# aurelienpierreeng/ansel

Hardware: AMD Instinct MI355X
Metric: MPix/s full export pixelpipe (100 MP raw); % MI355X HBM roofline (higher is better)
Workload: dtype f32

## Files before the change

### ansel_amd/csrc/diffuse.hip

```cpp
#include "hip_common.h"

#include <type_traits>
#include "devmath.h"
#include "ieee_inrange.h"
#include "px_colorspaces.h"

#include <math.h>
#include <cstdlib>

namespace ansel
{
int bspline_launch_decompose(int devid, hipStream_t s, const float4 *in, float4 *hf, float4 *lf, int w, int h, int mult,
                             const unsigned *gate = nullptr);
int bspline_launch_decompose3(int devid, hipStream_t s, const void *in, bool in4, float *lf, int w, int h, int mult, unsigned *alpha_flag);
#ifdef ANSEL_HIP_MEASURING
int bspline_launch_decompose2(int devid, hipStream_t s, const float4 *in, float4 *low1, float4 *low2, int w, int h, int mult);
#endif
}
using namespace ansel;

namespace
{

#define DIFFUSE_MAX_SCALES 10
#define BSPLINE_SIGMA 1.0553651328015339f
#define PDE_KAPPA 0.25f

__device__ __forceinline__ float max_first(const float a, const float b) { return a > b ? a : b; }
__device__ __forceinline__ float max_zero(const float v) { return isfinite(v) ? max_first(v, 0.0f) : 0.0f; }
__device__ __forceinline__ int clampi(const int v, const int lo, const int hi) { return v < lo ? lo : (v > hi ? hi : v); }

__device__ __forceinline__ int walk_row(const int b, const int height, const int mult)
{
  if(height <= mult) return b < height ? b : -1;
  const int per_pass = (height + mult - 1) / mult;
  const int row = (b % per_pass) * mult + b / per_pass;
  return row < height ? row : -1;
}

struct pde_args
{
  int width, height, mult;
  float anisotropy[4];
  int kind[4];
  int same02, same13;
  float variance_threshold, regularization;
  float abcd[4], strength;
  int wskip;
  int post_lab;
  float post_m[3][4];
  int approx_div;
  int off;
  const unsigned *gate;
  int gate_sense;
};

#ifdef ANSEL_HIP_MEASURING
#define PDE_APPROX(a) ((a).approx_div != 0)
#define PDE_OFF(a, bit) (((a).off & (bit)) != 0)
#else
#define PDE_APPROX(a) false
#define PDE_OFF(a, bit) false
#endif
__device__ __forceinline__ float div_1ulp(const float x, const float y)
{
  const float r = __builtin_amdgcn_rcpf(y);
  const float q = x * r;
  return __builtin_fmaf(__builtin_fmaf(-y, q, x), r, q);
}

__device__ __forceinline__ float fast_expf(const float x)
{
  const float t = 1065353216.0f + x * 11401300.0f;
  int k = (t > -2147483648.0f && t < 2147483648.0f) ? (int)t : 0;
  k = k > 0 ? k : 0;
  return __int_as_float(k);
}

__device__ __forceinline__ float direction(float gx, float gy, float &cos2, float &sin2, float &cs, const bool approx = false)
{
  const float s2 = gx * gx + gy * gy;
  float mag, inv;
  if(approx)
  {
    mag = __builtin_amdgcn_sqrtf(s2);
    inv = div_1ulp(1.0f, mag + (1.0f - ((mag != 0.0f) ? 1.0f : 0.0f)));
  }
  else if(__builtin_amdgcn_ballot_w64(!ansel_ieee::zero_or_above_2m96(s2)) == 0ull)
  {
    mag = ansel_ieee::sqrt_core(s2);
    inv = ansel_ieee::rcp_core(mag + (1.0f - ((mag != 0.0f) ? 1.0f : 0.0f)));
  }
  else
  {
    mag = sqrtf(s2);
    inv = 1.0f / (mag + (1.0f - ((mag != 0.0f) ? 1.0f : 0.0f)));
  }
  const float nonzero = (mag != 0.0f) ? 1.0f : 0.0f;
  gx = gx * inv + (1.0f - nonzero);
  gy = gy * inv;
  cos2 = gx * gx;
  sin2 = gy * gy;
  cs = gx * gy;
  return mag;
}

struct kernel5
{
  float k0, k1, k2, k3, k4;
};
__device__ __forceinline__ kernel5 order_kernel(const int kind, const float c2, const float cs, const float cos2, const float sin2)
{
  kernel5 w;
  if(kind == 0)
  {
    w.k0 = 0.25f; w.k1 = 0.5f; w.k2 = 0.25f; w.k3 = 0.5f; w.k4 = -3.0f;
  }
  else
  {
    float a00, a11, a01;
    if(kind == 1)
    {
      a00 = cos2 + c2 * sin2;
      a11 = c2 * cos2 + sin2;
      a01 = (c2 - 1.0f) * cs;
    }
    else
    {
      a00 = c2 * cos2 + sin2;
      a11 = cos2 + c2 * sin2;
      a01 = (1.0f - c2) * cs;
    }
    w.k0 = a01 * 0.5f;
    w.k1 = a11;
    w.k2 = -w.k0;
    w.k3 = a00;
    w.k4 = -2.0f * (a00 + a11);
  }
  return w;
}

__device__ __forceinline__ float convolve(const kernel5 w, const float p[9])
{
  float d = 0.0f;
  d = w.k0 * p[0] + d;
  d = w.k1 * p[1] + d;
  d = w.k2 * p[2] + d;
  d = w.k3 * p[3] + d;
  d = w.k4 * p[4] + d;
  d = w.k3 * p[5] + d;
  d = w.k2 * p[6] + d;
  d = w.k1 * p[7] + d;
  d = w.k0 * p[8] + d;
  return d;
}

__device__ __forceinline__ float ratio2(const float h, const float l)
{
  const float safe = max_zero(l - 1e-8f) + 1e-8f;
  const float ratio = h / safe;
  return ratio * ratio;
}
__device__ __forceinline__ float4 ratio2_rgb(const float4 h, const float4 l, const float w_ratio, const bool approx = false)
{
  if(approx)
  {
    const float ax = div_1ulp(h.x, max_zero(l.x - 1e-8f) + 1e-8f), ay = div_1ulp(h.y, max_zero(l.y - 1e-8f) + 1e-8f),
                az = div_1ulp(h.z, max_zero(l.z - 1e-8f) + 1e-8f);
    return make_float4(ax * ax, ay * ay, az * az, w_ratio);
  }
// ... 652 lines not shown
struct diffuse_planes_t
{
  dev_buf_t hf[DIFFUSE_MAX_SCALES], lf[2], tmp[2];
  dev_buf_t mask;
  dev_buf_t inpainted;
  dev_buf_t alpha_flag;
};

struct diffuse_job_t
{
  int devid;
  hipStream_t st;
  const dt_hip_diffuse_data_t *d;
  const dt_hip_lab_data_t *post_lab;
  int w, h, scales, iterations;
  float zoom;
  bool lf_chain;
  bool per_row, no_dma;
  diffuse_planes_t p;
};

static int diffuse_alloc_planes(diffuse_job_t &j, const bool in_place, const bool three)
{
  diffuse_planes_t &p = j.p;
  const size_t plane = (size_t)j.w * j.h * sizeof(float4);
  bool ok = true;
  for(int s = 0; s < j.scales; s++) ok &= (bool)(p.hf[s] = dev_buf_t::alloc(j.devid, plane));
  for(int k = 0; k < ((j.lf_chain && !in_place) ? 1 : 2); k++) ok &= (bool)(p.lf[k] = dev_buf_t::alloc(j.devid, plane));
  for(int k = 0; k < 2 && k < j.iterations - 1; k++) ok &= (bool)(p.tmp[k] = dev_buf_t::alloc(j.devid, plane));
  if(ok && three) ok &= (bool)(p.alpha_flag = dev_buf_t::alloc(j.devid, sizeof(unsigned)));
  if(ok && j.d->threshold > 0.0f)
  {
    p.mask = dev_buf_t::alloc(j.devid, (size_t)j.w * j.h);
    if(!p.tmp[1]) p.tmp[1] = dev_buf_t::alloc(j.devid, plane);
    p.inpainted = dev_buf_t::borrow(p.tmp[1].base());
    ok = p.mask && p.inpainted;
  }
  return ok ? DT_HIP_SUCCESS : DT_HIP_SYSMEM_ALLOCATION;
}

static void pde_args_of_call(pde_args &a, const int w, const int h, const dt_hip_diffuse_data_t *d)
{
  memset(&a, 0, sizeof(a));
  a.width = w;
  a.height = h;
  a.wskip = measuring_env("ANSEL_HIP_PDE_NO_WSKIP") ? 0 : 1;
  const char *const approx_env = measuring_env("ANSEL_HIP_PDE_APPROX_DIV");
  a.approx_div = approx_env && atoi(approx_env) != 0;
  const char *const off_env = measuring_env("ANSEL_HIP_PDE_OFF");
  a.off = off_env ? atoi(off_env) : 0;
  const float user_aniso[4] = { d->anisotropy_first, d->anisotropy_second, d->anisotropy_third, d->anisotropy_fourth };
  for(int k = 0; k < 4; k++)
  {
    a.anisotropy[k] = sqf(user_aniso[k]);
    a.kind[k] = user_aniso[k] == 0.0f ? 0 : (user_aniso[k] > 0.0f ? 1 : 2);
  }
  a.same02 = a.kind[0] == a.kind[2] && a.anisotropy[0] == a.anisotropy[2];
  a.same13 = a.kind[1] == a.kind[3] && a.anisotropy[1] == a.anisotropy[3];
  a.variance_threshold = powf(10.0f, d->variance_threshold);
}

static void pde_args_of_scale(pde_args &a, const diffuse_job_t &j, const int s, const bool last_pass)
{
  const dt_hip_diffuse_data_t *const d = j.d;
  const float regularization = powf(10.0f, d->regularization) - 1.0f;
  const float speed[4] = { d->first, d->second, d->third, d->fourth };
  const float real_radius = sigma_at_step(BSPLINE_SIGMA, (unsigned)s) * j.zoom;
  a.regularization = regularization / 9.0f * sqf(real_radius);
  const float norm = expf(-sqf(real_radius - (float)d->radius_center) / sqf((float)d->radius));
  for(int k = 0; k < 4; k++) a.abcd[k] = speed[k] * PDE_KAPPA * norm;
  a.strength = d->sharpness * norm + 1.0f;
  a.mult = 1 << s;
  a.post_lab = 0;
  if(j.post_lab && last_pass)
  {
    a.post_lab = 1;
    memcpy(a.post_m, j.post_lab->matrix, sizeof(a.post_m));
  }
}

typedef void (*pde_strip_fn)(const float4 *, const float4 *, const float4 *, float4 *, pde_args, int, const unsigned char *, int, int);
typedef void (*pde_strip3_fn)(const float4 *, const float4 *, const float4 *, float4 *, pde_args, int, int, int);

template <int MD> static pde_strip_fn pde_strip_forms(const bool chain, const bool dma)
{
  if(dma) return diffuse_pde_strip<true, MD, true>;
  if(chain) return diffuse_pde_strip<true, MD>;
  return diffuse_pde_strip<false, MD>;
}
static pde_strip_fn pde_strip_kernel(const int mode, const bool chain, const bool dma)
{
  switch(mode)
  {
#define PDE_CASE(MD) \
  case MD: return pde_strip_forms<MD>(chain, dma);
    PDE_MODES(PDE_CASE)
#undef PDE_CASE
    default: return pde_strip_forms<-1>(chain, dma);
  }
}
static pde_strip3_fn pde_strip3_kernel(const int mode, const bool h0_4)
{
  if(mode == PDE_MODE_DEBLUR) return h0_4 ? diffuse_pde_strip3<PDE_MODE_DEBLUR, true> : diffuse_pde_strip3<PDE_MODE_DEBLUR, false>;
  return h0_4 ? diffuse_pde_strip3<PDE_MODE_ISOTROPIC, true> : diffuse_pde_strip3<PDE_MODE_ISOTROPIC, false>;
}

static void pde_strip_launch(const diffuse_job_t &j, const pde_args &a, const bool p3, const bool h0_4, const bool chain,
                             const bool dma, const float4 *h0, const float4 *h1, const float4 *cur, float4 *to,
                             const int final_pass)
{
  const int w = j.w, h = j.h;
  const int classes = h < a.mult ? h : a.mult, per_class = (h + a.mult - 1) / a.mult;
  const int gx = (w + 255) / 256;
  int longest = 32;
#ifdef ANSEL_HIP_MEASURING
  static const char *const strip_env = measuring_env("ANSEL_HIP_PDE_STRIP");
  if(strip_env) longest = atoi(strip_env);
#endif
  const int strip = strip_rows(gx, classes, per_class, longest);
  const int spc = (per_class + strip - 1) / strip;
  size_t ring = (size_t)PDE_RING * (256 + 2 * a.mult) * sizeof(float4);
#ifdef ANSEL_HIP_MEASURING
  static const char *const pad_env = measuring_env("ANSEL_HIP_PDE_LDS_PAD");
  if(pad_env) ring += (size_t)atoi(pad_env);
#endif
  static const bool generic = measuring_env("ANSEL_HIP_PDE_GENERIC") != nullptr;
  const int mode = generic ? -1 : pde_mode_of(a);
  const dim3 sgrid(gx, classes * spc);
  if(p3)
  {
    const size_t lds3 = (size_t)PDE_RING * (256 + 2 * a.mult) * 12 + (size_t)4 * 3 * (64 + 2 * a.mult) * 16;
    pde_strip3_kernel(mode, h0_4)<<<sgrid, 256, lds3, j.st>>>(h0, h1, cur, to, a, final_pass, strip, spc);
    return;
  }
  const size_t lds = dma ? ring + (size_t)4 * 3 * (64 + 2 * a.mult) * sizeof(float4) : ring;
  pde_strip_kernel(mode, chain, dma)<<<sgrid, 256, lds, j.st>>>(h0, h1, cur, to, a, final_pass, j.p.mask.as<unsigned char>(), strip, spc);
}

static int diffuse_iteration(const diffuse_job_t &j, pde_args &a, const bool p3, const bool first, const bool last,
                             const float4 *src, float4 *dst)
{
  const int w = j.w, h = j.h, scales = j.scales;
  float4 *hf[DIFFUSE_MAX_SCALES];
  for(int s = 0; s < DIFFUSE_MAX_SCALES; s++) hf[s] = j.p.hf[s].as<float4>();
  float4 *const lf[2] = { j.p.lf[0].as<float4>(), j.p.lf[1].as<float4>() };
  unsigned *const alpha_flag = j.p.alpha_flag.as<unsigned>();
  const unsigned char *const mask = j.p.mask.as<unsigned char>();
  int err = DT_HIP_SUCCESS;
  const float4 *level = src;
  float4 *residual = lf[0];
  const bool chain = j.lf_chain && (const float4 *)dst != src;
  for(int s = 0; s < scales && err == DT_HIP_SUCCESS; s++)
  {
#ifdef ANSEL_HIP_MEASURING
    static const bool pairs = measuring_env("ANSEL_HIP_BSPLINE_PAIRS") != nullptr;
    if(chain && pairs && s + 1 < scales && (s == 0 || s == 2))
    {
      err = bspline_launch_decompose2(j.devid, j.st, level, hf[s], hf[s + 1], w, h, 1 << s);
      s++;
      level = residual = hf[s];
      continue;
    }
#endif
    float4 *low = chain ? hf[s] : lf[s % 2];
    if(p3) err = bspline_launch_decompose3(j.devid, j.st, level, first && s == 0, (float *)low, w, h, 1 << s, alpha_flag);
    else err = bspline_launch_decompose(j.devid, j.st, level, chain ? nullptr : hf[s], low, w, h, 1 << s, alpha_flag);
    level = low;
    residual = low;
  }
  float4 *pp[2] = { residual == lf[1] ? lf[0] : lf[1], residual };
  const float4 *cur = residual;
  int count = 0;
  for(int s = scales - 1; s >= 0 && err == DT_HIP_SUCCESS; s--, count++)
  {
    pde_args_of_scale(a, j, s, s == 0 && last);
    float4 *to = (s == 0) ? dst : (chain ? (count % 2 == 0 ? lf[0] : hf[s + 1]) : pp[count % 2]);
    {
      launch_scope ls(j.devid, "diffuse_pde");
      if(a.mult <= PDE_SHARED_MULT && !j.per_row)
      {
        const float4 *const h0 = chain ? (s == 0 ? src : hf[s - 1]) : hf[s], *const h1 = chain ? hf[s] : nullptr;
        const bool dma = chain && a.mult <= PDE_DMA_MAX_MULT && !j.no_dma;
        pde_strip_launch(j, a, p3, first && s == 0, chain, dma, h0, h1, cur, to, p3 ? (s == 0 && last) : s == 0);
      }
      else
      {
        const int rows = (h <= a.mult) ? h : ((h + a.mult - 1) / a.mult) * a.mult;
        const dim3 grid(xcd_pad((w + 255) / 256), rows);
        if(a.mult <= PDE_SHARED_MULT)
          diffuse_pde<true><<<grid, 256, (size_t)3 * (256 + 2 * a.mult) * sizeof(float4), j.st>>>(hf[s], cur, to, a, s == 0, mask);
        else
          diffuse_pde<false><<<grid, 256, 0, j.st>>>(hf[s], cur, to, a, s == 0, mask);
      }
    }
    err = check_launch("diffuse_pde");
    cur = to;
  }
  return err;
}

static int diffuse_run(int devid, const dt_hip_piece_t *piece, const dt_hip_diffuse_data_t *d, int first_row, dt_hip_mem_t dev_in,
                       dt_hip_mem_t dev_out, const dt_hip_lab_data_t *post_lab)
{
  if(!valid_device(devid) || !piece || !d || !dev_in || !dev_out) return DT_HIP_INVALID_ARG;
  if(piece->channels != 4)
  {
    set_last_error("diffuse: needs a 4-channel float input");
    return DT_HIP_INVALID_ARG;
  }
  const int w = piece->roi_out.width, h = piece->roi_out.height;
  if(w <= 0 || h <= 0) return DT_HIP_SUCCESS;
  if(!(d->iscale > 0.0f) || !(piece->roi_in.scale > 0.0)) return DT_HIP_INVALID_ARG;
  static const bool per_row_pde = measuring_env("ANSEL_HIP_PDE_PER_ROW") != nullptr;
  static const bool hf_planes = measuring_env("ANSEL_HIP_DIFFUSE_HF_PLANES") != nullptr;
  static const bool no_dma = measuring_env("ANSEL_HIP_PDE_NO_DMA") != nullptr;
  const int it_req = (int)ceilf((float)d->iterations);
  diffuse_job_t j;
  j.devid = devid;
  j.st = stream_of(devid);
  j.d = d;
  j.post_lab = post_lab;
  j.w = w, j.h = h;
  j.scales = scales_of(piece, d);
  j.iterations = it_req > 1 ? it_req : 1;
  j.zoom = (float)(d->iscale / piece->roi_in.scale);
  j.lf_chain = !per_row_pde && !hf_planes && (1 << (j.scales - 1)) <= PDE_SHARED_MULT;
  j.per_row = per_row_pde, j.no_dma = no_dma;
  const int iterations = j.iterations;
  pde_args a;
  pde_args_of_call(a, w, h, d);

  const int mode0 = pde_mode_of(a);
  const bool in_place = iterations == 1 && dev_in == dev_out && !(d->threshold > 0.0f);
  const bool three = j.lf_chain && !no_dma && !(d->threshold > 0.0f) && (1 << (j.scales - 1)) <= PDE_DMA_MAX_MULT &&
                     !(iterations == 1 && dev_in == dev_out) && !measuring_env("ANSEL_HIP_PDE_GENERIC") &&
                     (mode0 == PDE_MODE_DEBLUR || mode0 == PDE_MODE_ISOTROPIC);
  int err = diffuse_alloc_planes(j, in_place, three);
  unsigned *const alpha_flag = j.p.alpha_flag.as<unsigned>();
  if(err == DT_HIP_SUCCESS && alpha_flag && hipMemsetAsync(alpha_flag, 0, sizeof(unsigned), j.st) != hipSuccess) err = DT_HIP_DEFAULT_ERROR;
  const float4 *src = (const float4 *)dev_in;
  if(err == DT_HIP_SUCCESS && j.p.mask)
  {
    const size_t np = (size_t)w * h;
    launch_scope ls(devid, "diffuse_inpaint");
    diffuse_inpaint<<<pixel_grid(np), 256, 0, j.st>>>(src, j.p.inpainted.as<float4>(), j.p.mask.as<unsigned char>(), d->threshold, np,
                                                      (size_t)w, (size_t)first_row * w);
    err = check_launch("diffuse_inpaint");
    src = j.p.inpainted.as<float4>();
  }
  for(int seq = alpha_flag ? 0 : 1; seq < 2 && err == DT_HIP_SUCCESS; seq++)
  {
    const bool p3 = seq == 0;
    a.gate = alpha_flag;
    a.gate_sense = p3 ? 1 : 2;
    if(alpha_flag) src = (const float4 *)dev_in;
    for(int it = 0; err == DT_HIP_SUCCESS && it < iterations; it++)
    {
      float4 *dst = (it == iterations - 1) ? (float4 *)dev_out : j.p.tmp[it % 2].as<float4>();
      err = diffuse_iteration(j, a, p3, it == 0, it == iterations - 1, src, dst);
      src = dst;
    }
  }
  if(alpha_flag)
  {
    if(g_diffuse_probe && err == DT_HIP_SUCCESS
       && hipMemcpyAsync(g_diffuse_probe, alpha_flag, sizeof(unsigned), hipMemcpyDeviceToDevice, j.st) != hipSuccess)
      err = DT_HIP_DEFAULT_ERROR;
  }
  else if(g_diffuse_probe && err == DT_HIP_SUCCESS && hipMemsetAsync(g_diffuse_probe, 0xff, sizeof(unsigned), j.st) != hipSuccess)
    err = DT_HIP_DEFAULT_ERROR;
  return err;
}

}

extern "C" {

int dt_hip_test_diffuse_probe(void *sink)
{
  ansel::g_diffuse_probe = sink;
  return DT_HIP_SUCCESS;
}

void dt_hip_iop_diffuse_tiling(const dt_hip_piece_t *piece, const dt_hip_diffuse_data_t *d, dt_hip_tiling_t *tiling)
{
  const int scales = scales_of(piece, d);
  tiling->factor = 6.0625f + scales;
  tiling->factor_cl = 6.0625f + scales;
  tiling->maxbuf = 1.0f;
  tiling->maxbuf_cl = 1.0f;
  tiling->overhead = 0;
  tiling->overlap = 1 << scales;
  tiling->xalign = 1;
  tiling->yalign = 1;
}

}
```

### ansel_amd/csrc/diffuse_bspline.hip

```cpp
#include "hip_common.h"

#include <cstdlib>

using namespace ansel;

namespace
{

__device__ __forceinline__ float max_first(const float a, const float b) { return a > b ? a : b; }
__device__ __forceinline__ int clampi(const int v, const int lo, const int hi) { return v < lo ? lo : (v > hi ? hi : v); }

__device__ __forceinline__ float tap5(const float a, const float b, const float c, const float d, const float e)
{
  const float s = 0.0625f * a + 0.25f * b + 0.375f * c + 0.25f * d + 0.0625f * e;
  return max_first(0.0f, s);
}
__device__ __forceinline__ float4 tap5(const float4 a, const float4 b, const float4 c, const float4 d, const float4 e)
{
  return make_float4(tap5(a.x, b.x, c.x, d.x, e.x), tap5(a.y, b.y, c.y, d.y, e.y), tap5(a.z, b.z, c.z, d.z, e.z),
                     tap5(a.w, b.w, c.w, d.w, e.w));
}

__device__ __forceinline__ int walk_row(const int b, const int height, const int mult)
{
// ... 130 lines not shown
    if(more && own) n1 = in[BS_ROW(kk + 3) + col];
    if(more && second) n2 = in[BS_ROW(kk + 3) + col2];
    float4 *const V = vert[kk & 1];
    if(own) V[(k + 2) * R + r] = tap5(a, b, c, d, e);
    if(second) V[slot2] = tap5(a2, b2, c2, d2, e2);
    __syncthreads();
    if(own)
    {
      float4 t[5];
#pragma unroll
      for(int s = -2; s <= 2; s++)
      {
        const int cc = col + s * mult;
        t[s + 2] = cc < 0 ? V[(T + 4) * R] : (cc > width - 1 ? V[(T + 4) * R + 1] : V[(k + s + 2) * R + r]);
      }
      const float4 low = tap5(t[0], t[1], t[2], t[3], t[4]);
      const size_t o = (size_t)row * width + col;
      lf[o] = low;
      if(hf) nt_store(hf + o, make_float4(c.x - low.x, c.y - low.y, c.z - low.z, c.w - low.w));
    }
    a = b;
    b = c;
    c = d;
    d = e;
    e = n1;
    a2 = b2;
    b2 = c2;
    c2 = d2;
    d2 = e2;
    e2 = n2;
  }
#undef BS_ROW
}

struct bs_px3
{
  float x, y, z;
};
__device__ __forceinline__ bs_px3 tap5(const bs_px3 a, const bs_px3 b, const bs_px3 c, const bs_px3 d, const bs_px3 e)
{
  return { tap5(a.x, b.x, c.x, d.x, e.x), tap5(a.y, b.y, c.y, d.y, e.y), tap5(a.z, b.z, c.z, d.z, e.z) };
}
template <int R, int T, bool IN4>
__global__ __launch_bounds__(256) void bspline_decompose_strip3(const void *__restrict__ in_v, bs_px3 *__restrict__ lf,
                                                                const int width, const int height, const int strip,
                                                                const int strips_per_class, unsigned *__restrict__ alpha_flag)
{
  static_assert(R * T == 256, "a workgroup's columns: one span of 256");
  constexpr int mult = R;
  if(!IN4 && *alpha_flag != 0u) return;
  __shared__ bs_px3 vert[2][(T + 4) * R + 2];
  const float4 *const in4 = static_cast<const float4 *>(in_v);
  const bs_px3 *const in3 = static_cast<const bs_px3 *>(in_v);
  unsigned alpha_bits = 0;
  auto at = [&](const size_t i) -> bs_px3 {
    if constexpr(IN4)
    {
      const float4 v = in4[i];
      alpha_bits |= __float_as_uint(v.w);
      return { v.x, v.y, v.z };
    }
    else
      return in3[i];
  };
  const int cls = blockIdx.y / strips_per_class, k0s = (blockIdx.y - cls * strips_per_class) * strip;
  const int n_cls = (height - cls + mult - 1) / mult;
  if(k0s >= n_cls) return;
  const int nrows = (strip < n_cls - k0s) ? strip : n_cls - k0s;
  const int r_first = cls + k0s * mult;
  const int k0 = (int)blockIdx.x * T;
  const int tid = threadIdx.x;
  const int r = tid % R, k = tid / R;
  const int col = r + (k0 + k) * mult;
  const bool own = col < width;
  int col2 = -1, slot2 = 0;
  if(tid < 4 * R)
  {
    const int hr = tid % R, hs = tid / R;
    const int hk = hs < 2 ? hs - 2 : T + hs - 2;
    const int hcol = hr + (k0 + hk) * mult;
    if(hcol >= 0 && hcol < width)
    {
      col2 = hcol;
      slot2 = (hk + 2) * R + hr;
    }
  }
  else if(tid == 4 * R)
  {
    col2 = 0;
    slot2 = (T + 4) * R;
  }
  else if(tid == 4 * R + 1)
  {
    col2 = width - 1;
    slot2 = (T + 4) * R + 1;
  }
  const bool second = col2 >= 0;
#define BS_ROW(q) ((size_t)clampi(r_first + (q) * mult, 0, height - 1) * width)
  const bs_px3 z = { 0.f, 0.f, 0.f };
  bs_px3 a = z, b = z, c = z, d = z, e = z, a2 = z, b2 = z, c2 = z, d2 = z, e2 = z;
  if(own)
  {
    a = at(BS_ROW(-2) + col);
    b = at(BS_ROW(-1) + col);
    c = at(BS_ROW(0) + col);
    d = at(BS_ROW(1) + col);
    e = at(BS_ROW(2) + col);
  }
  if(second)
  {
    a2 = at(BS_ROW(-2) + col2);
    b2 = at(BS_ROW(-1) + col2);
    c2 = at(BS_ROW(0) + col2);
    d2 = at(BS_ROW(1) + col2);
    e2 = at(BS_ROW(2) + col2);
  }
  for(int kk = 0; kk < nrows; kk++)
  {
    const int row = r_first + kk * mult;
    const bool more = kk + 1 < nrows;
    bs_px3 n1 = z, n2 = z;
    if(more && own) n1 = at(BS_ROW(kk + 3) + col);
    if(more && second) n2 = at(BS_ROW(kk + 3) + col2);
    bs_px3 *const V = vert[kk & 1];
    if(own) V[(k + 2) * R + r] = tap5(a, b, c, d, e);
    if(second) V[slot2] = tap5(a2, b2, c2, d2, e2);
    __syncthreads();
    if(own)
    {
      bs_px3 t[5];
#pragma unroll
      for(int s = -2; s <= 2; s++)
      {
        const int cc = col + s * mult;
        t[s + 2] = cc < 0 ? V[(T + 4) * R] : (cc > width - 1 ? V[(T + 4) * R + 1] : V[(k + s + 2) * R + r]);
      }
      lf[(size_t)row * width + col] = tap5(t[0], t[1], t[2], t[3], t[4]);
    }
    a = b;
    b = c;
    c = d;
    d = e;
    e = n1;
    a2 = b2;
    b2 = c2;
    c2 = d2;
    d2 = e2;
    e2 = n2;
  }
#undef BS_ROW
  if(IN4 && __builtin_amdgcn_ballot_w64(alpha_bits != 0u) != 0ull && (tid & 63) == 0) atomicOr(alpha_flag, 1u);
}

#ifdef ANSEL_HIP_MEASURING
__device__ __forceinline__ float4 bs_row_taps(const float4 *__restrict__ V, const int col, const int step, const int origin,
                                              const int width)
{
  float4 t[5];
#pragma unroll
  for(int j = 0; j < 5; j++) t[j] = V[clampi(col + (j - 2) * step, 0, width - 1) - origin];
  return tap5(t[0], t[1], t[2], t[3], t[4]);
}

template <int M, int AHEAD>
__global__ __launch_bounds__(320) void bspline_decompose2_strip(const float4 *__restrict__ in, float4 *__restrict__ low1,
                                                                float4 *__restrict__ low2, const int width, const int height,
                                                                const int strip, const int strips_per_class)
{
  constexpr int M2 = 2 * M, WA = 256 + 12 * M, WB = 256 + 8 * M;
  static_assert(WA <= 320, "a lane a column");
  __shared__ float4 VA[2][WA], VC[2][WB];
  const int c0 = (int)blockIdx.x * 256;
  const int cls = blockIdx.y / strips_per_class, k0s = (blockIdx.y - cls * strips_per_class) * strip;
  const int n_cls = (height - cls + M2 - 1) / M2;
  if(k0s >= n_cls) return;
  const int nrows = (strip < n_cls - k0s) ? strip : n_cls - k0s;
  const int r_first = cls + k0s * M2;
  const int tid = threadIdx.x;
  const int ca = c0 - 6 * M + tid, cb = c0 - 4 * M + tid;
  const bool on_a = tid < WA && ca >= 0 && ca < width;
  const bool on_b = tid < WB && cb >= 0 && cb < width;
  const bool on_c = on_b && tid >= 4 * M && tid < 4 * M + 256;
  const float4 z = make_float4(0.f, 0.f, 0.f, 0.f);
  float4 a = z, b = z, c = z, d = z, e = z;
  float4 nd[AHEAD], ne[AHEAD];
  float4 r0 = z, r1 = z, r2 = z, r3 = z, r4 = z;
  bool rolling = false;
#define BS_AT(r) in[(size_t)clampi((r), 0, height - 1) * width + ca]
  const int ca_safe = clampi(ca, 0, width - 1);
#define BS_SAFE(r) in[(size_t)clampi((r), 0, height - 1) * width + ca_safe]
#pragma unroll
  for(int j = 0; j < AHEAD; j++)
  {
    const int sj = r_first + (j - 2) * M2;
    nd[j] = BS_SAFE(sj + M);
    ne[j] = BS_SAFE(sj + 2 * M);
  }
#define BS_STEP(kk, J) \
  { \
    const int k = (kk); \
    const int q = k + 5, sig = r_first + (q - 2) * M2, buf = q & 1; \
    const bool produce = q <= nrows + 3; \
    if(produce) \
    { \
      if(sig >= 0 && sig < height) \
      { \
        if(rolling) \
        { \
          a = c; \
          b = d; \
          c = e; \
        } \
        else \
        { \
          if(on_a) \
          { \
            a = BS_AT(sig - 2 * M); \
            b = BS_AT(sig - M); \
            c = BS_AT(sig); \
          } \
          rolling = true; \
        } \
        d = nd[J]; \
        e = ne[J]; \
        if(on_a) VA[buf][tid] = tap5(a, b, c, d, e); \
      } \
      else \
      { \
         \
        rolling = false; \
        const int tau = clampi(sig, 0, height - 1); \
        if(on_a) VA[buf][tid] = tap5(BS_AT(tau - 2 * M), BS_AT(tau - M), BS_AT(tau), BS_AT(tau + M), BS_AT(tau + 2 * M)); \
      } \
    } \
     \
    nd[J] = BS_SAFE(sig + AHEAD * M2 + M); \
    ne[J] = BS_SAFE(sig + AHEAD * M2 + 2 * M); \
    if(k >= 0 && on_b) VC[buf][tid] = tap5(r0, r1, r2, r3, r4); \
    __syncthreads(); \
    if(k >= 0 && on_c) low2[(size_t)(r_first + k * M2) * width + cb] = bs_row_taps(VC[buf], cb, M2, c0 - 4 * M, width); \
    if(produce) \
    { \
      r0 = r1; \
      r1 = r2; \
      r2 = r3; \
      r3 = r4; \
      if(on_b) \
      { \
        r4 = bs_row_taps(VA[buf], cb, M, c0 - 6 * M, width); \
        if(on_c && q >= 2 && q - 2 < nrows) low1[(size_t)sig * width + cb] = r4; \
      } \
    } \
  }
  for(int k0 = -5; k0 < nrows; k0 += AHEAD)
  {
    BS_STEP(k0, 0)
    if constexpr(AHEAD > 1)
      if(k0 + 1 < nrows) BS_STEP(k0 + 1, 1)
    if constexpr(AHEAD > 2)
      if(k0 + 2 < nrows) BS_STEP(k0 + 2, 2)
    if constexpr(AHEAD > 3)
      if(k0 + 3 < nrows) BS_STEP(k0 + 3, 3)
  }
#undef BS_STEP
#undef BS_AT
#undef BS_SAFE
}
#endif

}

namespace ansel
{
#ifdef ANSEL_HIP_MEASURING
int bspline_launch_decompose2(int devid, hipStream_t s, const float4 *in, float4 *low1, float4 *low2, int w, int h, int mult)
{
  (void)devid;
  if(mult != 1 && mult != 4) return DT_HIP_INVALID_ARG;
  const int m2 = 2 * mult;
  const int classes = h < m2 ? h : m2, per_class = (h + m2 - 1) / m2;
  const int gx = (w + 255) / 256;
  const int strip = strip_rows(gx, classes, per_class, 64);
  const int spc = (per_class + strip - 1) / strip;
  const dim3 grid(gx, classes * spc);
  launch_scope ls(devid, "diffuse_decompose");
  static const char *const ahead_env = measuring_env("ANSEL_HIP_BSPLINE_AHEAD");
  const int ahead = ahead_env ? atoi(ahead_env) : 1;
#define BS_PAIR(MM) \
  switch(ahead) \
  { \
    case 2: bspline_decompose2_strip<MM, 2><<<grid, 320, 0, s>>>(in, low1, low2, w, h, strip, spc); break; \
    case 4: bspline_decompose2_strip<MM, 4><<<grid, 320, 0, s>>>(in, low1, low2, w, h, strip, spc); break; \
    case 3: bspline_decompose2_strip<MM, 3><<<grid, 320, 0, s>>>(in, low1, low2, w, h, strip, spc); break; \
    default: bspline_decompose2_strip<MM, 1><<<grid, 320, 0, s>>>(in, low1, low2, w, h, strip, spc); break; \
  }
  if(mult == 1)
  {
    BS_PAIR(1);
  }
  else
  {
    BS_PAIR(4);
  }
#undef BS_PAIR
  return check_launch("diffuse_decompose");
}
#endif

int bspline_launch_decompose3(int devid, hipStream_t s, const void *in, bool in4, float *lf, int w, int h, int mult, unsigned *alpha_flag)
{
  (void)devid;
  if(mult != 1 && mult != 2 && mult != 4 && mult != 8 && mult != 16) return DT_HIP_INVALID_ARG;
  if(in4 && mult != 1) return DT_HIP_INVALID_ARG;
  const int classes = h < mult ? h : mult, per_class = (h + mult - 1) / mult;
  const int gx = (w + 255) / 256;
  const int strip = strip_rows(gx, classes, per_class);
  const int spc = (per_class + strip - 1) / strip;
  const dim3 grid(gx, classes * spc);
  launch_scope ls(devid, "diffuse_decompose");
  bs_px3 *const out = reinterpret_cast<bs_px3 *>(lf);
  if(in4) bspline_decompose_strip3<1, 256, true><<<grid, 256, 0, s>>>(in, out, w, h, strip, spc, alpha_flag);
  else if(mult == 1) bspline_decompose_strip3<1, 256, false><<<grid, 256, 0, s>>>(in, out, w, h, strip, spc, alpha_flag);
  else if(mult == 2) bspline_decompose_strip3<2, 128, false><<<grid, 256, 0, s>>>(in, out, w, h, strip, spc, alpha_flag);
  else if(mult == 4) bspline_decompose_strip3<4, 64, false><<<grid, 256, 0, s>>>(in, out, w, h, strip, spc, alpha_flag);
  else if(mult == 8) bspline_decompose_strip3<8, 32, false><<<grid, 256, 0, s>>>(in, out, w, h, strip, spc, alpha_flag);
  else bspline_decompose_strip3<16, 16, false><<<grid, 256, 0, s>>>(in, out, w, h, strip, spc, alpha_flag);
  return check_launch("diffuse_decompose");
}

int bspline_launch_decompose(int devid, hipStream_t s, const float4 *in, float4 *hf, float4 *lf, int w, int h, int mult,
                             const unsigned *gate)
{
  const int steps = (w + mult - 1) / mult;
  launch_scope ls(devid, "diffuse_decompose");
#ifdef ANSEL_HIP_MEASURING
  static const bool per_row = getenv("ANSEL_HIP_BSPLINE_PER_ROW") != nullptr;
  if(per_row)
  {
    const int rows = (h <= mult) ? h : ((h + mult - 1) / mult) * mult;
    if(mult == 1)
      bspline_decompose<1, 256><<<dim3(xcd_pad((steps + 255) / 256), rows), 256, 0, s>>>(in, hf, lf, w, h, mult, 1, (steps + 255) / 256);
    else if(mult == 2)
      bspline_decompose<2, 128><<<dim3(xcd_pad((steps + 127) / 128), rows), 256, 0, s>>>(in, hf, lf, w, h, mult, 1, (steps + 127) / 128);
    else if(mult == 4)
      bspline_decompose<4, 64><<<dim3(xcd_pad((steps + 63) / 64), rows), 256, 0, s>>>(in, hf, lf, w, h, mult, 1, (steps + 63) / 64);
    else
    {
      const int groups = mult / 8;
      bspline_decompose<8, 32><<<dim3(xcd_pad(((steps + 31) / 32) * groups), rows), 256, 0, s>>>(in, hf, lf, w, h, mult, groups,
                                                                                            ((steps + 31) / 32) * groups);
    }
    return check_launch("diffuse_decompose");
  }
#endif
  const int classes = h < mult ? h : mult, per_class = (h + mult - 1) / mult;
  const int gx = mult == 1 ? (steps + 255) / 256 : (mult == 2 ? (steps + 127) / 128 : (mult == 4 ? (steps + 63) / 64 : ((steps + 31) / 32) * (mult / 8)));
  const int strip = strip_rows(gx, classes, per_class);
  const int spc = (per_class + strip - 1) / strip;
  const dim3 grid(gx, classes * spc);
  if(mult == 1) bspline_decompose_strip<1, 256><<<grid, 256, 0, s>>>(in, hf, lf, w, h, mult, 1, strip, spc, gate);
  else if(mult == 2) bspline_decompose_strip<2, 128><<<grid, 256, 0, s>>>(in, hf, lf, w, h, mult, 1, strip, spc, gate);
  else if(mult == 4) bspline_decompose_strip<4, 64><<<grid, 256, 0, s>>>(in, hf, lf, w, h, mult, 1, strip, spc, gate);
  else bspline_decompose_strip<8, 32><<<grid, 256, 0, s>>>(in, hf, lf, w, h, mult, mult / 8, strip, spc, gate);
  return check_launch("diffuse_decompose");
}
}
```

### ansel_amd/csrc/hip_common.h

```cpp
#pragma once
#include <hip/hip_runtime.h>
#include <stdint.h>
#include <stdio.h>
#include <string.h>
#include "ansel_hip.h"
#include "dev_buf.h"

#ifdef ANSEL_HIP_MEASURING
#include <stdlib.h>
static inline const char *measuring_env(const char *name) { return getenv(name); }
#else
static inline constexpr const char *measuring_env(const char *) { return nullptr; }
#endif

namespace ansel
{

enum dispatch_key_t
{
  DISPATCH_NLM_V2 = 0,
  DISPATCH_NLM_FUSED,
  DISPATCH_AMAZE_UNFUSED,
  DISPATCH_AMAZE_SLAB,
  DISPATCH_AMAZE_BLOCKS,
  DISPATCH_BILAT_BLUR_SPLIT,
  DISPATCH_STRIP_ROWS,
  DISPATCH_KEYS
};
int dispatch_override(dispatch_key_t key);

static inline int strip_rows(const int gx, const int classes, const int per_class, const int longest = 32)
{
  const int forced = dispatch_override(DISPATCH_STRIP_ROWS);
  if(forced) return forced;
  int strip = longest;
  while(strip > 4 && (size_t)gx * classes * ((per_class + strip - 1) / strip) < 2048) strip /= 2;
  return strip;
}

void set_last_error(const char *fmt, ...);

hipStream_t stream_of(int devid);
int upload_small(int devid, void *dst_dev, const void *src_host, size_t bytes);
bool make_current(int devid);
int hip_device_of(int devid);
bool valid_device(int devid);

struct launch_scope
{
  int devid;
  const char *tag;
  hipEvent_t start, stop;
  bool active;
  launch_scope(int devid, const char *tag);
  ~launch_scope();
};

static inline int check_launch(const char *what)
{
  const hipError_t e = hipGetLastError();
  if(e != hipSuccess)
  {
    set_last_error("%s: %s", what, hipGetErrorString(e));
    return DT_HIP_DEFAULT_ERROR;
  }
  return DT_HIP_SUCCESS;
}

#define ANSEL_HIP_CHECK(expr)                                                                   \
  do                                                                                            \
  {                                                                                             \
    const hipError_t _e = (expr);                                                               \
    if(_e != hipSuccess)                                                                        \
    {                                                                                           \
      ansel::set_last_error("%s:%d %s: %s", __FILE__, __LINE__, #expr, hipGetErrorString(_e));  \
      return DT_HIP_DEFAULT_ERROR;                                                              \
    }                                                                                           \
  } while(0)

typedef float v4f_t __attribute__((ext_vector_type(4)));
__device__ __forceinline__ void nt_store(float4 *p, const float4 v)
{
  const v4f_t t = { v.x, v.y, v.z, v.w };
  __builtin_nontemporal_store(t, reinterpret_cast<v4f_t *>(p));
}

template <typename T> __device__ __forceinline__ const T &kernarg_at(const int offset)
{
  typedef const T __attribute__((address_space(4))) *p4;
  return *(const T *)(p4)((const char __attribute__((address_space(4))) *)__builtin_amdgcn_kernarg_segment_ptr() + offset);
}
template <typename T, typename... Before> constexpr int kernarg_offset_after()
{
  size_t off = 0;
  ((off = (off + alignof(Before) - 1) / alignof(Before) * alignof(Before) + sizeof(Before)), ...);
  return (int)((off + alignof(T) - 1) / alignof(T) * alignof(T));
}

static inline unsigned xcd_pad(const int gx) { return (unsigned)((gx + 7) / 8) * 8; }
__device__ __forceinline__ int xcd_col() { return (int)((blockIdx.x + blockIdx.y / 64) % gridDim.x); }

#define HL_MIN_CLIPPED 25
struct hl_journal
{
  unsigned long long count;
  unsigned long long index[HL_MIN_CLIPPED];
  float value[HL_MIN_CLIPPED];
};
int highlights_resolve_launch(int devid, float *out, const hl_journal *journal);

struct rcd_band_t
{
  int tv0, tv1;
  int in_row0, in_rows;
  int out_row0, out_rows;
};

struct band_view_t
{
  int frame_h;
  int buf_row0;
  int row0, row1;
};
int nlmeans_halo_rows(const dt_hip_piece_t *piece, const dt_hip_nlmeans_data_t *d);
int nlmeans_process_band(int devid, const dt_hip_piece_t *piece, const dt_hip_nlmeans_data_t *d, const band_view_t *band,
                         dt_hip_mem_t dev_in, dt_hip_mem_t dev_out);
int diffuse_halo_rows(const dt_hip_piece_t *piece, const dt_hip_diffuse_data_t *d);
int diffuse_process_rows(int devid, const dt_hip_piece_t *piece, const dt_hip_diffuse_data_t *d, int first_row,
                         dt_hip_mem_t dev_in, dt_hip_mem_t dev_out);
int diffuse_process_post_lab(int devid, const dt_hip_piece_t *piece, const dt_hip_diffuse_data_t *d, dt_hip_mem_t dev_in,
                             dt_hip_mem_t dev_out, const dt_hip_lab_data_t *lab);
int denoiseprofile_halo_rows(const dt_hip_piece_t *piece, const dt_hip_denoiseprofile_data_t *d);
struct dn_band_job_t;
int denoiseprofile_band_begin(int devid, const dt_hip_piece_t *piece, const dt_hip_denoiseprofile_data_t *d,
                              const band_view_t *band, int buf_rows, dt_hip_mem_t dev_in, dt_hip_mem_t dev_out,
                              dn_band_job_t **job);
int denoiseprofile_band_step(dn_band_job_t *job, dt_hip_mem_t *halo_buf, int *halo_rows, double **sums, size_t *sum_count);
int denoiseprofile_band_finish(dn_band_job_t *job, dt_hip_mem_t dev_out);
void denoiseprofile_band_abort(dn_band_job_t *job);
int guided_filter_launch(int devid, const float4 *guide, float *mask, int width, int height, int w, float sqrt_eps,
                         float guide_weight, float minv, float maxv);
int detail_refine_launch(int devid, const float *rawdetail, const float *form, float fill, float level, int width, int height,
                         float *refined);
int bilat_band_supported(const dt_hip_piece_t *piece, const dt_hip_bilat_data_t *d);
int blend_refines_with_detail_mask(const dt_hip_blend_data_t *d);
int bilat_band_begin(int devid, const dt_hip_piece_t *piece, const dt_hip_bilat_data_t *d, dt_hip_mem_t *grid, size_t *bytes);
int bilat_band_splat(int devid, const dt_hip_piece_t *piece, const dt_hip_bilat_data_t *d, dt_hip_mem_t grid,
                     dt_hip_mem_t in_rows, int row0, int rows);
int bilat_band_finish(int devid, const dt_hip_piece_t *piece, const dt_hip_bilat_data_t *d, dt_hip_mem_t grid,
                      dt_hip_mem_t in_rows, dt_hip_mem_t out_rows, int row0, int rows);

int file_host_view(const char *who, int devid, void *host, size_t host_bytes, void **view);
int file_to_host_launch(hipStream_t s, const void *dev_file, size_t capacity, void *view, size_t host_bytes);

static inline unsigned stream_grid(size_t work_items, unsigned block)
{
  size_t g = (work_items + block - 1) / block;
  if(g > 2048u * 4u) g = 2048u * 4u;
  if(g < 1) g = 1;
  return (unsigned)g;
}

static inline unsigned pixel_grid(size_t pixels)
{
  const size_t g = (pixels + 255) / 256;
  return (unsigned)(g < 1 ? 1 : (g > 0x7fffffffu ? 0x7fffffffu : g));
}

}
```

### ansel_amd/csrc/testhooks.hip

```cpp
#include "hip_common.h"
#include "devmath.h"
#include "ieee_inrange.h"

#include <atomic>
#include <string.h>

using namespace ansel;

namespace
{
std::atomic<int> g_dispatch[DISPATCH_KEYS];
const char *const g_dispatch_names[DISPATCH_KEYS] = { "nlm_v2", "nlm_fused", "amaze_unfused", "amaze_slab", "amaze_blocks",
                                                       "bilat_blur_split", "strip_rows" };
}
namespace ansel
{
int dispatch_override(const dispatch_key_t key) { return g_dispatch[key].load(std::memory_order_relaxed); }
}
extern "C" int dt_hip_test_dispatch(const char *key, int value)
{
  if(!key) return DT_HIP_INVALID_ARG;
  for(int k = 0; k < DISPATCH_KEYS; k++)
    if(!strcmp(key, g_dispatch_names[k]))
    {
      if(k == DISPATCH_STRIP_ROWS && value != 0 && value != 4 && value != 8 && value != 16 && value != 32) return DT_HIP_INVALID_ARG;
      g_dispatch[k].store(value);
      return DT_HIP_SUCCESS;
    }
  return DT_HIP_INVALID_ARG;
}

extern "C" int dt_hip_test_strip_rows(int gx, int classes, int per_class) { return strip_rows(gx, classes, per_class); }

namespace
{
template <int FN>
__global__ void devmath_test(const float *__restrict__ x, const float *__restrict__ y, float *__restrict__ o, const size_t n)
{
  for(size_t k = (size_t)blockIdx.x * blockDim.x + threadIdx.x; k < n; k += (size_t)gridDim.x * blockDim.x)
  {
    float r;
    if(FN == 0) r = ansel_math::powf_exact(x[k], y[k]);
    else if(FN == 1) r = ansel_math::log2f_exact(x[k]);
    else if(FN == 2) r = ansel_math::exp2f_exact(x[k]);
    else if(FN == 3) r = ansel_math::expf_exact(x[k]);
    else if(FN == 4) r = ansel_math::atan2f_exact(x[k], y[k]);
    else if(FN == 5) r = ansel_math::hypotf_exact(x[k], y[k]);
    else if(FN == 6) r = ansel_math::sinf_exact(x[k]);
    else if(FN == 7) r = ansel_math::cosf_exact(x[k]);
    else if(FN == 9) r = ansel_math::logf_exact(x[k]);
    else if(FN == 10) r = ansel_ieee::div_core(x[k], y[k]);
    else if(FN == 11) r = ansel_ieee::rcp_core(x[k]);
    else if(FN == 12) r = ansel_ieee::sqrt_core(x[k]);
    else if(FN == 13) r = ansel_ieee::zero_or_above_2m96(x[k]) ? 1.0f : 0.0f;
    else if(FN == 14) r = ansel_ieee::div_uniform(x[k], y[k], ansel_ieee::rcp_refined(y[k]));
    else r = fmodf(x[k], y[k]);
    o[k] = r;
  }
}
template <int FN> int devmath_launch(int devid, const void *x, const void *y, void *o, size_t n)
{
  if(!valid_device(devid)) return DT_HIP_INVALID_ARG;
  devmath_test<FN><<<stream_grid(n, 256), 256, 0, stream_of(devid)>>>((const float *)x, (const float *)y, (float *)o, n);
  return check_launch("devmath_test");
}
}
extern "C" {
int dt_hip_test_powf(int devid, const void *x, const void *y, void *o, size_t n) { return devmath_launch<0>(devid, x, y, o, n); }
int dt_hip_test_log2f(int devid, const void *x, const void *y, void *o, size_t n) { return devmath_launch<1>(devid, x, y, o, n); }
int dt_hip_test_exp2f(int devid, const void *x, const void *y, void *o, size_t n) { return devmath_launch<2>(devid, x, y, o, n); }
int dt_hip_test_expf(int devid, const void *x, const void *y, void *o, size_t n) { return devmath_launch<3>(devid, x, y, o, n); }
int dt_hip_test_atan2f(int devid, const void *x, const void *y, void *o, size_t n) { return devmath_launch<4>(devid, x, y, o, n); }
int dt_hip_test_hypotf(int devid, const void *x, const void *y, void *o, size_t n) { return devmath_launch<5>(devid, x, y, o, n); }
int dt_hip_test_sinf(int devid, const void *x, const void *y, void *o, size_t n) { return devmath_launch<6>(devid, x, y, o, n); }
int dt_hip_test_cosf(int devid, const void *x, const void *y, void *o, size_t n) { return devmath_launch<7>(devid, x, y, o, n); }
int dt_hip_test_fmodf(int devid, const void *x, const void *y, void *o, size_t n) { return devmath_launch<8>(devid, x, y, o, n); }
int dt_hip_test_logf(int devid, const void *x, const void *y, void *o, size_t n) { return devmath_launch<9>(devid, x, y, o, n); }
int dt_hip_test_div_core(int devid, const void *x, const void *y, void *o, size_t n) { return devmath_launch<10>(devid, x, y, o, n); }
int dt_hip_test_rcp_core(int devid, const void *x, const void *y, void *o, size_t n) { return devmath_launch<11>(devid, x, y, o, n); }
int dt_hip_test_sqrt_core(int devid, const void *x, const void *y, void *o, size_t n) { return devmath_launch<12>(devid, x, y, o, n); }
int dt_hip_test_zero_or_above_2m96(int devid, const void *x, const void *y, void *o, size_t n) { return devmath_launch<13>(devid, x, y, o, n); }
int dt_hip_test_div_uniform(int devid, const void *x, const void *y, void *o, size_t n) { return devmath_launch<14>(devid, x, y, o, n); }
}

namespace
{
__global__ __launch_bounds__(64) void lds_dma_x3_test(const float *__restrict__ src, unsigned *__restrict__ dst, const unsigned base)
{
  __shared__ unsigned lds[512];
  for(int i = threadIdx.x; i < 512; i += 64) lds[i] = 0xdeadbeefu;
  __syncthreads();
  using lds_u32_ptr = __attribute__((address_space(3))) unsigned *;
  const unsigned m0v = (unsigned)__builtin_amdgcn_readfirstlane((int)(unsigned)(__UINTPTR_TYPE__)(lds_u32_ptr)lds) + base;
  const unsigned voff = (63u - threadIdx.x) * 12u;
  unsigned keep;
  asm volatile("s_waitcnt lgkmcnt(0)\n\ts_nop 4\n\ts_mov_b32 %0, m0\n\t"
               "s_mov_b32 m0, %3\n\ts_nop 0\n\tglobal_load_lds_dwordx3 %1, %2\n\t"
               "s_mov_b32 m0, %0\n\ts_waitcnt vmcnt(0)"
               : "=&s"(keep)
               : "v"(voff), "s"(src), "s"(m0v)
               : "memory");
  __syncthreads();
  for(int i = threadIdx.x; i < 512; i += 64) dst[i] = lds[i];
}
}
extern "C" int dt_hip_test_lds_dma_x3(int devid, const void *src, void *dst, unsigned base)
{
  if(!valid_device(devid) || !src || !dst || base % 4 != 0 || base + 1024 > 2048) return DT_HIP_INVALID_ARG;
  lds_dma_x3_test<<<1, 64, 0, stream_of(devid)>>>((const float *)src, (unsigned *)dst, base);
  return check_launch("lds_dma_x3_test");
}
```

Before: 1649.

## Fuse paired B-spline decomposition scales into one 3-channel kernel by default

Replaces the measurement-only float4 two-scale B-spline kernel with a production 3-channel (bs_px3) version. By default it computes scales 0/1 and 2/3 in a single launch, keeping the intermediate level in LDS instead of re-reading it from HBM. Edge rows are precomputed into an LDS buffer, and the alpha flag is checked and set the same way as in the single-scale kernel. This cuts launches and memory traffic for the wavelet decomposition. In exchange it adds LDS pressure, extra halo recomputation and barrier-heavy stepping, and a dispatch override can turn it off.

```diff
diff --git a/ansel_amd/csrc/diffuse.hip b/ansel_amd/csrc/diffuse.hip
--- a/ansel_amd/csrc/diffuse.hip
+++ b/ansel_amd/csrc/diffuse.hip
@@ -13,9 +13,8 @@
 int bspline_launch_decompose(int devid, hipStream_t s, const float4 *in, float4 *hf, float4 *lf, int w, int h, int mult,
                              const unsigned *gate = nullptr);
 int bspline_launch_decompose3(int devid, hipStream_t s, const void *in, bool in4, float *lf, int w, int h, int mult, unsigned *alpha_flag);
-#ifdef ANSEL_HIP_MEASURING
-int bspline_launch_decompose2(int devid, hipStream_t s, const float4 *in, float4 *low1, float4 *low2, int w, int h, int mult);
-#endif
+int bspline_launch_decompose_pair3(int devid, hipStream_t s, const void *in, bool in4, float *low1, float *low2, int w, int h,
+                                   int mult, unsigned *alpha_flag);
 }
 using namespace ansel;
 
@@ -974,16 +973,14 @@
   const bool chain = j.lf_chain && (const float4 *)dst != src;
   for(int s = 0; s < scales && err == DT_HIP_SUCCESS; s++)
   {
-#ifdef ANSEL_HIP_MEASURING
-    static const bool pairs = measuring_env("ANSEL_HIP_BSPLINE_PAIRS") != nullptr;
-    if(chain && pairs && s + 1 < scales && (s == 0 || s == 2))
-    {
-      err = bspline_launch_decompose2(j.devid, j.st, level, hf[s], hf[s + 1], w, h, 1 << s);
+    if(p3 && chain && s + 1 < scales && (s == 0 || s == 2) && !dispatch_override(DISPATCH_BSPLINE_SINGLE))
+    {
+      err = bspline_launch_decompose_pair3(j.devid, j.st, level, first && s == 0, (float *)hf[s], (float *)hf[s + 1], w, h, 1 << s,
+                                           alpha_flag);
       s++;
       level = residual = hf[s];
       continue;
     }
-#endif
     float4 *low = chain ? hf[s] : lf[s % 2];
     if(p3) err = bspline_launch_decompose3(j.devid, j.st, level, first && s == 0, (float *)low, w, h, 1 << s, alpha_flag);
     else err = bspline_launch_decompose(j.devid, j.st, level, chain ? nullptr : hf[s], low, w, h, 1 << s, alpha_flag);
diff --git a/ansel_amd/csrc/diffuse_bspline.hip b/ansel_amd/csrc/diffuse_bspline.hip
--- a/ansel_amd/csrc/diffuse_bspline.hip
+++ b/ansel_amd/csrc/diffuse_bspline.hip
@@ -306,161 +306,119 @@
   if(IN4 && __builtin_amdgcn_ballot_w64(alpha_bits != 0u) != 0ull && (tid & 63) == 0) atomicOr(alpha_flag, 1u);
 }
 
-#ifdef ANSEL_HIP_MEASURING
-__device__ __forceinline__ float4 bs_row_taps(const float4 *__restrict__ V, const int col, const int step, const int origin,
-                                              const int width)
-{
-  float4 t[5];
+__device__ __forceinline__ bs_px3 bs_row_taps3(const bs_px3 *__restrict__ V, const int col, const int step, const int origin,
+                                               const int width)
+{
+  bs_px3 t[5];
 #pragma unroll
   for(int j = 0; j < 5; j++) t[j] = V[clampi(col + (j - 2) * step, 0, width - 1) - origin];
   return tap5(t[0], t[1], t[2], t[3], t[4]);
 }
 
-template <int M, int AHEAD>
-__global__ __launch_bounds__(320) void bspline_decompose2_strip(const float4 *__restrict__ in, float4 *__restrict__ low1,
-                                                                float4 *__restrict__ low2, const int width, const int height,
-                                                                const int strip, const int strips_per_class)
-{
-  constexpr int M2 = 2 * M, WA = 256 + 12 * M, WB = 256 + 8 * M;
+template <bool IN4> struct bs_raw
+{
+  typedef bs_px3 type;
+};
+template <> struct bs_raw<true>
+{
+  typedef float4 type;
+};
+
+template <int M, bool IN4>
+__global__ __launch_bounds__(320, 5) void bspline_decompose_pair3(const void *__restrict__ in_v, bs_px3 *__restrict__ low1,
+                                                               bs_px3 *__restrict__ low2, const int width, const int height,
+                                                               const int strip, const int strips_per_class,
+                                                               unsigned *__restrict__ alpha_flag)
+{
+  constexpr int WA = 256 + 12 * M, WB = 256 + 8 * M;
   static_assert(WA <= 320, "a lane a column");
-  __shared__ float4 VA[2][WA], VC[2][WB];
+  if(!IN4 && *alpha_flag != 0u) return;
+  __shared__ bs_px3 VA[2][WA], VC[2][WB], EDGE[2][WB];
+  typedef typename bs_raw<IN4>::type raw_t;
+  const raw_t *const in = static_cast<const raw_t *>(in_v);
+  unsigned alpha_bits = 0;
+  auto take = [&](const raw_t v) -> bs_px3 {
+    if constexpr(IN4) alpha_bits |= __float_as_uint(v.w);
+    return { v.x, v.y, v.z };
+  };
   const int c0 = (int)blockIdx.x * 256;
   const int cls = blockIdx.y / strips_per_class, k0s = (blockIdx.y - cls * strips_per_class) * strip;
-  const int n_cls = (height - cls + M2 - 1) / M2;
+  const int n_cls = (height - cls + M - 1) / M;
   if(k0s >= n_cls) return;
-  const int nrows = (strip < n_cls - k0s) ? strip : n_cls - k0s;
-  const int r_first = cls + k0s * M2;
+  const int k1s = k0s + ((strip < n_cls - k0s) ? strip : n_cls - k0s);
   const int tid = threadIdx.x;
   const int ca = c0 - 6 * M + tid, cb = c0 - 4 * M + tid;
   const bool on_a = tid < WA && ca >= 0 && ca < width;
   const bool on_b = tid < WB && cb >= 0 && cb < width;
   const bool on_c = on_b && tid >= 4 * M && tid < 4 * M + 256;
-  const float4 z = make_float4(0.f, 0.f, 0.f, 0.f);
-  float4 a = z, b = z, c = z, d = z, e = z;
-  float4 nd[AHEAD], ne[AHEAD];
-  float4 r0 = z, r1 = z, r2 = z, r3 = z, r4 = z;
-  bool rolling = false;
-#define BS_AT(r) in[(size_t)clampi((r), 0, height - 1) * width + ca]
   const int ca_safe = clampi(ca, 0, width - 1);
-#define BS_SAFE(r) in[(size_t)clampi((r), 0, height - 1) * width + ca_safe]
-#pragma unroll
-  for(int j = 0; j < AHEAD; j++)
-  {
-    const int sj = r_first + (j - 2) * M2;
-    nd[j] = BS_SAFE(sj + M);
-    ne[j] = BS_SAFE(sj + 2 * M);
-  }
-#define BS_STEP(kk, J) \
-  { \
-    const int k = (kk); \
-    const int q = k + 5, sig = r_first + (q - 2) * M2, buf = q & 1; \
-    const bool produce = q <= nrows + 3; \
-    if(produce) \
-    { \
-      if(sig >= 0 && sig < height) \
-      { \
-        if(rolling) \
-        { \
-          a = c; \
-          b = d; \
-          c = e; \
-        } \
-        else \
-        { \
-          if(on_a) \
-          { \
-            a = BS_AT(sig - 2 * M); \
-            b = BS_AT(sig - M); \
-            c = BS_AT(sig); \
-          } \
-          rolling = true; \
-        } \
-        d = nd[J]; \
-        e = ne[J]; \
-        if(on_a) VA[buf][tid] = tap5(a, b, c, d, e); \
-      } \
-      else \
-      { \
-         \
-        rolling = false; \
-        const int tau = clampi(sig, 0, height - 1); \
-        if(on_a) VA[buf][tid] = tap5(BS_AT(tau - 2 * M), BS_AT(tau - M), BS_AT(tau), BS_AT(tau + M), BS_AT(tau + 2 * M)); \
-      } \
-    } \
-     \
-    nd[J] = BS_SAFE(sig + AHEAD * M2 + M); \
-    ne[J] = BS_SAFE(sig + AHEAD * M2 + 2 * M); \
-    if(k >= 0 && on_b) VC[buf][tid] = tap5(r0, r1, r2, r3, r4); \
-    __syncthreads(); \
-    if(k >= 0 && on_c) low2[(size_t)(r_first + k * M2) * width + cb] = bs_row_taps(VC[buf], cb, M2, c0 - 4 * M, width); \
-    if(produce) \
-    { \
-      r0 = r1; \
-      r1 = r2; \
-      r2 = r3; \
-      r3 = r4; \
-      if(on_b) \
-      { \
-        r4 = bs_row_taps(VA[buf], cb, M, c0 - 6 * M, width); \
-        if(on_c && q >= 2 && q - 2 < nrows) low1[(size_t)sig * width + cb] = r4; \
-      } \
-    } \
-  }
-  for(int k0 = -5; k0 < nrows; k0 += AHEAD)
-  {
-    BS_STEP(k0, 0)
-    if constexpr(AHEAD > 1)
-      if(k0 + 1 < nrows) BS_STEP(k0 + 1, 1)
-    if constexpr(AHEAD > 2)
-      if(k0 + 2 < nrows) BS_STEP(k0 + 2, 2)
-    if constexpr(AHEAD > 3)
-      if(k0 + 3 < nrows) BS_STEP(k0 + 3, 3)
-  }
-#undef BS_STEP
-#undef BS_AT
-#undef BS_SAFE
-}
-#endif
+  auto frame_row = [&](const int r) -> raw_t { return in[(size_t)clampi(r, 0, height - 1) * width + ca_safe]; };
+  const bs_px3 z = { 0.f, 0.f, 0.f };
+  auto edge_row = [&](const int tau) -> bs_px3 {
+    const bs_px3 v = tap5(take(frame_row(tau - 2 * M)), take(frame_row(tau - M)), take(frame_row(tau)), take(frame_row(tau + M)),
+                          take(frame_row(tau + 2 * M)));
+    if(on_a) VA[0][tid] = v;
+    __syncthreads();
+    bs_px3 r = z;
+    if(on_b) r = bs_row_taps3(VA[0], cb, M, c0 - 6 * M, width);
+    __syncthreads();
+    return r;
+  };
+  const int t0 = k0s - 4, t1 = k1s + 3;
+  if(t0 < 0)
+  {
+    const bs_px3 r = edge_row(0);
+    if(tid < WB) EDGE[0][tid] = r;
+  }
+  if(t1 >= n_cls)
+  {
+    const bs_px3 r = edge_row(height - 1);
+    if(tid < WB) EDGE[1][tid] = r;
+  }
+  const int v_last = t1 + 2;
+  auto class_row = [&](const int v) -> raw_t { return frame_row(cls + (v < v_last ? v : v_last) * M); };
+  bs_px3 a = take(class_row(t0 - 2)), b = take(class_row(t0 - 1)), c = take(class_row(t0)), d = take(class_row(t0 + 1)),
+         e = take(class_row(t0 + 2));
+  raw_t q0 = class_row(t0 + 3), q1 = class_row(t0 + 4);
+  bs_px3 P[5] = { z, z, z, z, z }, Q[5] = { z, z, z, z, z };
+  auto step = [&](const int t, const int buf, const bs_px3(&RD)[5], bs_px3(&WR)[5], raw_t &slot) {
+    const bool make1 = t <= t1 && t >= 0 && t < n_cls;
+    const bool make2 = t - 5 >= k0s && t - 5 < k1s;
+    if(make1 && on_a) VA[buf][tid] = tap5(a, b, c, d, e);
+    if(make2 && on_b) VC[buf][tid] = tap5(RD[0], RD[1], RD[2], RD[3], RD[4]);
+    __syncthreads();
+    bs_px3 r = z;
+    if(!(t >= 0 && t < n_cls) && t <= t1 && tid < WB) r = EDGE[t < 0 ? 0 : 1][tid];
+    if(make1 && on_b)
+    {
+      r = bs_row_taps3(VA[buf], cb, M, c0 - 6 * M, width);
+      if(on_c && t >= k0s && t < k1s) low1[(size_t)(cls + t * M) * width + cb] = r;
+    }
+    if(make2 && on_c) low2[(size_t)(cls + (t - 5) * M) * width + cb] = bs_row_taps3(VC[buf], cb, 2 * M, c0 - 4 * M, width);
+    WR[0] = WR[1];
+    WR[1] = WR[2];
+    WR[2] = WR[3];
+    WR[3] = WR[4];
+    WR[4] = r;
+    a = b;
+    b = c;
+    c = d;
+    d = e;
+    e = take(slot);
+    slot = class_row(t + 5);
+  };
+  for(int t = t0; t <= t1 + 1; t += 2)
+  {
+    step(t, 0, Q, P, q0);
+    step(t + 1, 1, P, Q, q1);
+  }
+  if(IN4 && __builtin_amdgcn_ballot_w64(alpha_bits != 0u) != 0ull && (tid & 63) == 0) atomicOr(alpha_flag, 1u);
+}
 
 }
 
 namespace ansel
 {
-#ifdef ANSEL_HIP_MEASURING
-int bspline_launch_decompose2(int devid, hipStream_t s, const float4 *in, float4 *low1, float4 *low2, int w, int h, int mult)
-{
-  (void)devid;
-  if(mult != 1 && mult != 4) return DT_HIP_INVALID_ARG;
-  const int m2 = 2 * mult;
-  const int classes = h < m2 ? h : m2, per_class = (h + m2 - 1) / m2;
-  const int gx = (w + 255) / 256;
-  const int strip = strip_rows(gx, classes, per_class, 64);
-  const int spc = (per_class + strip - 1) / strip;
-  const dim3 grid(gx, classes * spc);
-  launch_scope ls(devid, "diffuse_decompose");
-  static const char *const ahead_env = measuring_env("ANSEL_HIP_BSPLINE_AHEAD");
-  const int ahead = ahead_env ? atoi(ahead_env) : 1;
-#define BS_PAIR(MM) \
-  switch(ahead) \
-  { \
-    case 2: bspline_decompose2_strip<MM, 2><<<grid, 320, 0, s>>>(in, low1, low2, w, h, strip, spc); break; \
-    case 4: bspline_decompose2_strip<MM, 4><<<grid, 320, 0, s>>>(in, low1, low2, w, h, strip, spc); break; \
-    case 3: bspline_decompose2_strip<MM, 3><<<grid, 320, 0, s>>>(in, low1, low2, w, h, strip, spc); break; \
-    default: bspline_decompose2_strip<MM, 1><<<grid, 320, 0, s>>>(in, low1, low2, w, h, strip, spc); break; \
-  }
-  if(mult == 1)
-  {
-    BS_PAIR(1);
-  }
-  else
-  {
-    BS_PAIR(4);
-  }
-#undef BS_PAIR
-  return check_launch("diffuse_decompose");
-}
-#endif
-
 int bspline_launch_decompose3(int devid, hipStream_t s, const void *in, bool in4, float *lf, int w, int h, int mult, unsigned *alpha_flag)
 {
   (void)devid;
@@ -482,6 +440,24 @@
   return check_launch("diffuse_decompose");
 }
 
+int bspline_launch_decompose_pair3(int devid, hipStream_t s, const void *in, bool in4, float *low1, float *low2, int w, int h,
+                                   int mult, unsigned *alpha_flag)
+{
+  (void)devid;
+  if((mult != 1 && mult != 4) || (in4 && mult != 1)) return DT_HIP_INVALID_ARG;
+  const int classes = h < mult ? h : mult, per_class = (h + mult - 1) / mult;
+  const int gx = (w + 255) / 256;
+  const int strip = strip_rows(gx, classes, per_class, 128);
+  const int spc = (per_class + strip - 1) / strip;
+  const dim3 grid(gx, classes * spc);
+  launch_scope ls(devid, "diffuse_decompose");
+  bs_px3 *const o1 = reinterpret_cast<bs_px3 *>(low1), *const o2 = reinterpret_cast<bs_px3 *>(low2);
+  if(in4) bspline_decompose_pair3<1, true><<<grid, 320, 0, s>>>(in, o1, o2, w, h, strip, spc, alpha_flag);
+  else if(mult == 1) bspline_decompose_pair3<1, false><<<grid, 320, 0, s>>>(in, o1, o2, w, h, strip, spc, alpha_flag);
+  else bspline_decompose_pair3<4, false><<<grid, 320, 0, s>>>(in, o1, o2, w, h, strip, spc, alpha_flag);
+  return check_launch("diffuse_decompose");
+}
+
 int bspline_launch_decompose(int devid, hipStream_t s, const float4 *in, float4 *hf, float4 *lf, int w, int h, int mult,
                              const unsigned *gate)
 {
diff --git a/ansel_amd/csrc/hip_common.h b/ansel_amd/csrc/hip_common.h
--- a/ansel_amd/csrc/hip_common.h
+++ b/ansel_amd/csrc/hip_common.h
@@ -25,6 +25,7 @@
   DISPATCH_AMAZE_BLOCKS,
   DISPATCH_BILAT_BLUR_SPLIT,
   DISPATCH_STRIP_ROWS,
+  DISPATCH_BSPLINE_SINGLE,
   DISPATCH_KEYS
 };
 int dispatch_override(dispatch_key_t key);
diff --git a/ansel_amd/csrc/testhooks.hip b/ansel_amd/csrc/testhooks.hip
--- a/ansel_amd/csrc/testhooks.hip
+++ b/ansel_amd/csrc/testhooks.hip
@@ -11,7 +11,7 @@
 {
 std::atomic<int> g_dispatch[DISPATCH_KEYS];
 const char *const g_dispatch_names[DISPATCH_KEYS] = { "nlm_v2", "nlm_fused", "amaze_unfused", "amaze_slab", "amaze_blocks",
-                                                       "bilat_blur_split", "strip_rows" };
+                                                       "bilat_blur_split", "strip_rows", "bspline_single" };
 }
 namespace ansel
 {
```

New measurement: 1664 (median of 6 runs). Within noise of the previous version (+1.0%).
